# IBM/VillanDiffusion

Measured on AMD Instinct MI355X. Metric: train imgs/sec + 1000-step DDPM sample imgs/sec, CIFAR10 bs128, higher is better.
Workload: dtype bf16x3/f32; 1 GPU; DDPM-CIFAR10-32 poisoned fine-tune B=128 (BOX_14->HAT pr0.1 SDE-VP) + DDPM-1000 sampling 1024 img/GPU (8x128, 4 streams); global_batch=128, image=3x32x32, parallelism=dp1, mode=all, full=False

## Files before the change

include/villan_hip.h:

```cpp
#ifndef VILLAN_HIP_H
#define VILLAN_HIP_H

#include <stdint.h>

#ifdef __cplusplus
extern "C" {
#endif

#define VD_ABI_VERSION 11
#define VD_EINVAL (-22)
#define VD_ETIMEDOUT (-110)

int vd_abi_version(void);
const char* vd_last_error(void);
int vd_device_ok(void);
int vd_async_errors(int clear);

enum vd_a_mode { VD_A_ROW = 0,
                 VD_A_COL = 1 };
enum vd_b_mode { VD_B_PLAIN = 0,
                 VD_B_KCONTIG = 1,
                 VD_B_CONV3 = 2,
                 VD_B_CONV3_T = 3,
                 VD_B_CONV3_S2 = 4,
// ... 64 lines not shown
} vd_wgrad_desc;

int vd_conv_wgrad(const vd_wgrad_desc* desc, void* stream);
int64_t vd_conv_wgrad_ws_floats(const vd_wgrad_desc* desc);
int vd_conv_wgrad_plan(const vd_wgrad_desc* desc, int* tile, int* splits);

int vd_presplit_pack(const float* x, void* y, int B, int C, int HW, int64_t x_bstride, int64_t y_bstride, void* stream);
int vd_presplit_unpack(const void* y, float* x, int B, int C, int HW, int64_t y_bstride, int64_t x_bstride, void* stream);
int vd_groupnorm_fwd_presplit_ok(int C, int HW, int G);
int vd_groupnorm_fwd_presplit(const float* x, const float* gamma, const float* beta, void* y, float* mean, float* rstd, int B, int C, int HW, int G,
                              float eps, int apply_silu, int64_t x_bstride, int64_t y_bstride, void* stream);
int vd_groupnorm_bwd_presplit(const float* dy, const float* x, const float* mean, const float* rstd, const float* gamma, const float* beta,
                              const float* extra, const float* extra2, float* dx, void* dx_ps, float* dgamma_ws, float* dbeta_ws, float* rowsum,
                              int B, int C, int HW, int G, int apply_silu, int64_t dy_bstride, int64_t x_bstride, int64_t extra_bstride,
                              int64_t extra2_bstride, int64_t dx_bstride, int64_t ps_bstride, int64_t rowsum_ld, void* stream);

int vd_conv_wgrad_group_class(const vd_wgrad_desc* desc);
int64_t vd_conv_wgrad_group_job_bytes(void);
int vd_conv_wgrad_group_variant(int cls);
int vd_conv_wgrad_group_plan(const vd_wgrad_desc* descs, int n, void* table_out, int64_t* ws_floats, int* blocks, int* rblocks);
int vd_conv_wgrad_group_rebase(void* dev_table, int n, float* ws, void* stream);
int vd_conv_wgrad_group_launch(const void* dev_table, int n, int cls, int blocks, int rblocks, void* stream);

int64_t vd_conv3_packed_bytes(int M, int C, int taps);
int vd_conv3_pack_weights(const float* W, void* packed, int M, int C, int taps, int64_t row_stride, int64_t chan_stride, void* stream);
int vd_conv3_pack_weights_multi(const int64_t* table, int n_jobs, int64_t total_blocks, void* stream);
int vd_conv3_pack_weights_f16_multi(const int64_t* table, int n_jobs, int64_t total_blocks, void* stream);

int vd_weight_transpose(const float* W, float* Wt, int M, int C, int T, void* stream);
int vd_sumpool2x2(const float* dU, float* dX, int B, int C, int H, int W, int64_t du_bstride, int64_t dx_bstride,
                  int accumulate, void* stream);
int vd_col2im_s2(const float* G, float* dX, int B, int C, int H, int W, int OH, int OW, int pad, int64_t g_bstride,
                 int64_t dx_bstride, void* stream);
int vd_rowsum(const float* X, float* ws, int B, int M, int P, int64_t x_bstride, int64_t ws_ld, void* stream);
int vd_colsum(const float* ws, float* out, int B, int C, int64_t ld, int accumulate, void* stream);
int vd_colsum_segmented(const int64_t* table, int n_jobs, int B, void* stream);

int64_t vd_groupnorm_ws_floats(int B, int C, int HW, int G);
int vd_groupnorm_fwd(const float* x, const float* gamma, const float* beta, float* y, float* mean, float* rstd,
                     int B, int C, int HW, int G, float eps, int apply_silu, int64_t x_bstride, int64_t y_bstride,
                     float* ws, void* stream);
int vd_groupnorm_stats(const float* x, const float* gamma, const float* beta, float* ss, float* mean, float* rstd,
                       int B, int C, int HW, int G, float eps, int64_t x_bstride, void* stream);
int vd_groupnorm_stats_from_partials(const float* part, int tiles, const float* gamma, const float* beta, float* ss, float* mean,
                                     float* rstd, int B, int C, int HW, int G, float eps, void* stream);
int vd_groupnorm_bwd(const float* dy, const float* x, const float* mean, const float* rstd, const float* gamma,
                     const float* beta, const float* extra, float* dx, float* dgamma_ws, float* dbeta_ws,
                     int B, int C, int HW, int G, int apply_silu, int64_t dy_bstride, int64_t x_bstride,
                     int64_t extra_bstride, int64_t dx_bstride, float* ws, void* stream);
int vd_groupnorm_bwd_fused(const float* dy, const float* x, const float* mean, const float* rstd, const float* gamma,
                           const float* beta, const float* extra, const float* extra2, float* dx, float* dgamma_ws,
                           float* dbeta_ws, float* rowsum, int B, int C, int HW, int G, int apply_silu,
                           int64_t dy_bstride, int64_t x_bstride, int64_t extra_bstride, int64_t extra2_bstride,
                           int64_t dx_bstride, int64_t rowsum_ld, float* ws, void* stream);

int vd_softmax_col_fwd(float* S, int nb, int N, void* stream);
int vd_softmax_col_bwd(const float* P, float* dP, int nb, int N, float scale, void* stream);
int vd_attn_small_fwd(const float* qkv, float* out, float* P, int B, int C, int N, float scale,
                      int64_t qkv_bstride, int64_t out_bstride, void* stream);
int vd_attn_small_bwd(const float* qkv, const float* P, const float* dout, float* dqkv, int B, int C, int N,
                      float scale, int64_t qkv_bstride, int64_t dout_bstride, int64_t dqkv_bstride, void* stream);

int vd_attn_core_fwd(const float* qkv, float* out, float* P, int B, int heads, int head_dim, int N, float scale, void* stream);
int vd_attn_core_bwd(const float* qkv, const float* P, const float* out, const float* dout, float* dS, float* dqkv, int B, int heads,
                     int head_dim, int N, float scale, void* stream);

// ... 73 lines not shown
```

villandiffusion_amd/lib.py:

```python
from __future__ import annotations

import ctypes as C
import os
import subprocess
from typing import Optional

_HERE = os.path.dirname(os.path.abspath(__file__))
LIB_PATH = os.path.join(_HERE, "libvillan_hip.so")
CSRC = os.path.join(_HERE, "csrc")

A_ROW, A_COL = 0, 1
B_PLAIN, B_KCONTIG, B_CONV3, B_CONV3_T, B_CONV3_S2, B_CONV3_UP, B_CONV3_DIL, B_CONVG = range(8)

_i32, _i64, _f32, _vp = C.c_int32, C.c_int64, C.c_float, C.c_void_p


class GemmDesc(C.Structure):
    _fields_ = [("A", _vp), ("B", _vp), ("D", _vp), ("bias", _vp), ("rowadd", _vp), ("residual", _vp),
                ("M", _i32), ("N", _i32), ("K", _i32), ("a_mode", _i32), ("b_mode", _i32), ("NP", _i32),
                ("C", _i32), ("H", _i32), ("W", _i32), ("OH", _i32), ("OW", _i32),
                ("bias_on_n", _i32), ("d_trans", _i32), ("accumulate", _i32), ("tile", _i32), ("debug", _i32), ("alpha", _f32),
                ("lda", _i64), ("a_bstride", _i64), ("ldb", _i64), ("b_bstride", _i64),
                ("ldd", _i64), ("d_bstride", _i64), ("res_bstride", _i64), ("rowadd_bstride", _i64), ("ws", _vp), ("pad", _i32), ("nb2", _i32),
                ("a_b2stride", _i64), ("b_b2stride", _i64), ("d_b2stride", _i64), ("gn_ss", _vp), ("a_packed", _vp), ("a_packed_mpad", _i32), ("math", _i32), ("pool2", _i32),
# ... 8 lines not shown
                ("mode", _i32), ("splits", _i32), ("accumulate", _i32), ("tile", _i32),
                ("dy_bstride", _i64), ("x_bstride", _i64), ("pad", _i32), ("math", _i32), ("presplit", _i32), ("reserved_", _i32)]


PROTOTYPES = {
    "vd_abi_version": (_i32, []),
    "vd_last_error": (C.c_char_p, []),
    "vd_async_errors": (_i32, [_i32]),
    "vd_device_ok": (_i32, []),
    "vd_gemm": (_i32, [C.POINTER(GemmDesc), _vp]),
    "vd_gemm_tile": (_i32, [C.POINTER(GemmDesc)]),
    "vd_gemm_ws_floats": (_i64, [C.POINTER(GemmDesc)]),
    "vd_conv_wgrad": (_i32, [C.POINTER(WgradDesc), _vp]),
    "vd_conv_wgrad_plan": (_i32, [C.POINTER(WgradDesc), C.POINTER(_i32), C.POINTER(_i32)]),
    "vd_conv_wgrad_ws_floats": (_i64, [C.POINTER(WgradDesc)]),
    "vd_presplit_pack": (_i32, [_vp, _vp, _i32, _i32, _i32, _i64, _i64, _vp]),
    "vd_presplit_unpack": (_i32, [_vp, _vp, _i32, _i32, _i32, _i64, _i64, _vp]),
    "vd_groupnorm_fwd_presplit_ok": (_i32, [_i32, _i32, _i32]),
    "vd_groupnorm_fwd_presplit": (_i32, [_vp, _vp, _vp, _vp, _vp, _vp, _i32, _i32, _i32, _i32, _f32, _i32, _i64, _i64, _vp]),
    "vd_groupnorm_bwd_presplit": (_i32, [_vp] * 12 + [_vp, _i32, _i32, _i32, _i32, _i32] + [_i64] * 7 + [_vp]),
    "vd_conv_wgrad_group_class": (_i32, [C.POINTER(WgradDesc)]),
    "vd_conv_wgrad_group_job_bytes": (_i64, []),
    "vd_conv_wgrad_group_variant": (_i32, [_i32]),
    "vd_conv_wgrad_group_plan": (_i32, [C.POINTER(WgradDesc), _i32, _vp, C.POINTER(_i64), C.POINTER(_i32), C.POINTER(_i32)]),
    "vd_conv_wgrad_group_rebase": (_i32, [_vp, _i32, _vp, _vp]),
    "vd_conv_wgrad_group_launch": (_i32, [_vp, _i32, _i32, _i32, _i32, _vp]),
    "vd_conv3_packed_bytes": (_i64, [_i32, _i32, _i32]),
    "vd_conv3_pack_weights": (_i32, [_vp, _vp, _i32, _i32, _i32, _i64, _i64, _vp]),
    "vd_conv3_pack_weights_multi": (_i32, [_vp, _i32, _i64, _vp]),
    "vd_conv3_pack_weights_f16_multi": (_i32, [_vp, _i32, _i64, _vp]),
    "vd_weight_transpose": (_i32, [_vp, _vp, _i32, _i32, _i32, _vp]),
    "vd_sumpool2x2": (_i32, [_vp, _vp, _i32, _i32, _i32, _i32, _i64, _i64, _i32, _vp]),
    "vd_col2im_s2": (_i32, [_vp, _vp, _i32, _i32, _i32, _i32, _i32, _i32, _i32, _i64, _i64, _vp]),
    "vd_rowsum": (_i32, [_vp, _vp, _i32, _i32, _i32, _i64, _i64, _vp]),
    "vd_colsum": (_i32, [_vp, _vp, _i32, _i32, _i64, _i32, _vp]),
    "vd_colsum_segmented": (_i32, [_vp, _i32, _i32, _vp]),
    "vd_groupnorm_ws_floats": (_i64, [_i32, _i32, _i32, _i32]),
    "vd_groupnorm_stats": (_i32, [_vp, _vp, _vp, _vp, _vp, _vp, _i32, _i32, _i32, _i32, _f32, _i64, _vp]),
    "vd_groupnorm_fwd": (_i32, [_vp, _vp, _vp, _vp, _vp, _vp, _i32, _i32, _i32, _i32, _f32, _i32, _i64, _i64, _vp, _vp]),
    "vd_groupnorm_bwd": (_i32, [_vp] * 10 + [_i32] * 5 + [_i64] * 4 + [_vp, _vp]),
    "vd_groupnorm_stats_from_partials": (_i32, [_vp, _i32, _vp, _vp, _vp, _vp, _vp, _i32, _i32, _i32, _i32, _f32, _vp]),
    "vd_groupnorm_bwd_fused": (_i32, [_vp] * 12 + [_i32] * 5 + [_i64] * 6 + [_vp, _vp]),
    "vd_softmax_col_fwd": (_i32, [_vp, _i32, _i32, _vp]),
    "vd_softmax_col_bwd": (_i32, [_vp, _vp, _i32, _i32, _f32, _vp]),
    "vd_attn_small_fwd": (_i32, [_vp, _vp, _vp, _i32, _i32, _i32, _f32, _i64, _i64, _vp]),
    "vd_attn_small_bwd": (_i32, [_vp, _vp, _vp, _vp, _i32, _i32, _i32, _f32, _i64, _i64, _i64, _vp]),
    "vd_attn_core_fwd": (_i32, [_vp, _vp, _vp, _i32, _i32, _i32, _i32, _f32, _vp]),
    "vd_attn_core_bwd": (_i32, [_vp, _vp, _vp, _vp, _vp, _vp, _i32, _i32, _i32, _i32, _f32, _vp]),
    "vd_attn_flash_fwd": (_i32, [_vp, _vp, _vp, _i32, _i32, _i32, _i32, _f32, _i64, _i64, _vp]),
    "vd_attn_flash_bwd": (_i32, [_vp, _vp, _vp, _vp, _vp, _vp, _i32, _i32, _i32, _i32, _f32, _i64, _i64, _i64, _i64, _vp]),
    "vd_timestep_embedding": (_i32, [_vp, _vp, _vp, _i32, _i32, _i32, _vp]),
    "vd_silu_fwd": (_i32, [_vp, _vp, _i64, _vp]),
    "vd_silu_bwd": (_i32, [_vp, _vp, _vp, _i64, _i32, _vp]),
    "vd_add_strided": (_i32, [_vp, _vp, _i32, _i64, _i64, _i64, _i32, _vp]),
    "vd_scale": (_i32, [_vp, _i64, _f32, _vp]),
    "vd_lincomb": (_i32, [_vp, C.POINTER(_vp), C.POINTER(_f32), _i32, _i64, _vp]),
    "vd_qsample_backdoor": (_i32, [_vp] * 10 + [_i32, _i64, _vp]),
    "vd_mse_fwd_bwd": (_i32, [_vp] * 6 + [_i32, _i64, _f32, _vp]),
    "vd_loss_fwd_bwd": (_i32, [_vp] * 6 + [_i32, _i64, _f32, _i32, _vp]),
    "vd_trigger_inv_objective": (_i32, [_vp, _vp, _f32, _vp, _vp, _vp, _vp, _i32, _i64, _i64, _vp]),
    "vd_removal_loss": (_i32, [_vp, _vp, _f32, _f32, _f32, _vp, _vp, _vp, _i32, _i64, _i64, _vp]),
    "vd_score_inv_objective": (_i32, [_vp, _vp, _f32, _f32, _vp, _vp, _vp, _vp, _i32, _i64, _i64, _vp]),
    "vd_image_set_stats": (_i32, [_vp, _i32, _i32, _i32, _i32, _i64, _f32, _f32, _f32, _f32, _vp, _vp, _vp, _vp]),
    "vd_image_set_merge": (_i32, [_vp, _vp, _i64, _vp, _vp, _i64, _i64, _vp, _vp]),
    "vd_l2norm_sq": (_i32, [_vp, _i64, _vp, _vp, _vp]),
    "vd_adam_step": (_i32, [_vp, _vp, _vp, _vp, _i64, _vp, _f32, _f32, _f32, _f32, _f32, _f32, _i32, _vp, _vp]),
# ... 82 lines not shown
```

villandiffusion_amd/ops.py:

```python
from __future__ import annotations

import ctypes as C
import math
import os
from typing import Optional, Sequence

import torch

from . import lib as L
from .lib import (A_COL, A_ROW, B_CONV3, B_CONV3_DIL, B_CONVG, B_CONV3_S2, B_CONV3_T, B_CONV3_UP, B_KCONTIG, B_PLAIN,
                  GemmDesc, WgradDesc)


def _lib():
    L.require_device()
    return L.load()


_PROF = None

_B_NAMES = {0: "PLAIN", 1: "KCONTIG", 2: "CONV3", 3: "CONV3_T", 4: "CONV3_S2", 5: "CONV3_UP", 6: "CONV3_DIL", 7: "CONVG"}
_TILE_NAMES = {1: "128x128", 2: "64x128", 3: "64x64", 4: "patch128x128"}


# ... 651 lines not shown
        return (OH * OW) % 8 == 0 and M >= 64 and Cc >= 64
    if (mode == B_CONV3 and OW == 4 and OH == 4) or (mode in (B_CONV3, B_CONV3_UP) and OW >= 64 and OW % 32 == 0):
        return M >= 64 and Cc >= 64
    if mode == B_CONV3_S2:
        return OH == OW and (OW in (8, 16, 32) or (OW >= 64 and OW % 32 == 0)) and M >= 64 and Cc >= 64 and _wgrad_s2_split(OW)
    return mode in (B_CONV3, B_CONV3_UP) and OH == OW and OW in (8, 16, 32) and M >= 64 and Cc >= 64


def wgrad_ws_floats(M, Cc, T, nb, NP, OH=None, OW=None, mode=None, math_mode=0) -> int:
    d = WgradDesc()
    if OH is None:
        OH = OW = int(round(math.sqrt(NP)))
    d.M, d.C, d.T, d.nb, d.NP, d.OH, d.OW = M, Cc, T, nb, NP, OH, OW
    d.mode = (B_PLAIN if T == 1 else B_CONV3) if mode is None else mode
    d.math = math_mode
    scale = {B_CONV3_UP: (1, 2), B_CONV3_S2: (2, 1)}.get(d.mode, (1, 1))
    d.H, d.W = OH * scale[0] // scale[1], OW * scale[0] // scale[1]
    return int(L.load().vd_conv_wgrad_ws_floats(C.byref(d)))


def weight_transpose(w2d, wt, M, Cc, T):
    L.check(_lib().vd_weight_transpose(_p(w2d), _p(wt), M, Cc, T, _s()), "vd_weight_transpose")
    return wt


def sumpool2x2(dU, dX, accumulate=False):
    Bn, Cc, H, W, xbs = _img(dX)
    ubs = _img(dU)[4]
    assert dU.shape == (Bn, Cc, 2 * H, 2 * W)
    L.check(_lib().vd_sumpool2x2(_p(dU), _p(dX), Bn, Cc, H, W, ubs, xbs, int(accumulate), _s()), "vd_sumpool2x2")
    return dX


def conv3x3_s2_dgrad(dy, w2d, dx, pad=0, a_packed=None):
    Bn, M, OH, OW, dbs = _img(dy)
    Bx, Cc, H, W, xbs = _img(dx)
    assert Bx == Bn and w2d.shape == (M, Cc * 9) and w2d.is_contiguous()
    OHW = OH * OW
    G = torch.empty((Bn, Cc * 9, OHW), device=dy.device, dtype=torch.float32)
    gemm(w2d, dy, G, M=Cc * 9, N=Bn * OHW, K=M, a_mode=A_COL, b_mode=B_PLAIN, NP=OHW, lda=Cc * 9, ldb=OHW, b_bstride=dbs,
         ldd=OHW, d_bstride=Cc * 9 * OHW, a_packed=a_packed)
    L.check(_lib().vd_col2im_s2(_p(G), _p(dx), Bn, Cc, H, W, OH, OW, pad, Cc * 9 * OHW, xbs, _s()), "vd_col2im_s2")
    return dx


def rowsum(x, ws, ws_ld=None):
    Bn, M, H, W, xbs = _img(x)
    ld = M if ws_ld is None else ws_ld
    L.check(_lib().vd_rowsum(_p(x), _p(ws), Bn, M, H * W, xbs, ld, _s()), "vd_rowsum")
    return ws


def colsum(ws, out, Bn, Cc, ld=None, accumulate=False):
    L.check(_lib().vd_colsum(_p(ws), _p(out), Bn, Cc, Cc if ld is None else ld, int(accumulate), _s()), "vd_colsum")
    return out


def colsum_segmented(table, n_jobs, Bn):
    assert table.dtype == torch.int64 and table.is_contiguous() and table.numel() >= 4 * n_jobs
    L.check(_lib().vd_colsum_segmented(_p(table), n_jobs, Bn, _s()), "vd_colsum_segmented")


def _gn_ws(Bn, Cc, HW, G, device):
    need = _lib().vd_groupnorm_ws_floats(Bn, Cc, HW, G)
    return _gemm_ws(need, device) if need > 0 else None


def groupnorm_fwd(x, gamma, beta, y, mean, rstd, G, eps, silu):
    Bn, Cc, H, W, xbs = _img(x)
    ybs = _img(y)[4]
    assert y.shape == x.shape and mean.numel() >= Bn * G and rstd.numel() >= Bn * G
    _timed("groupnorm_fwd (gn_fwd_reg_kernel<*> / gn_chunk_*)", 8.0 * x.numel(), "hbm", lambda: L.check(
        _lib().vd_groupnorm_fwd(_p(x), _p(gamma), _p(beta), _p(y), _p(mean), _p(rstd), Bn, Cc, H * W, G, eps,
                                int(silu), xbs, ybs, _p(_gn_ws(Bn, Cc, H * W, G, x.device)), _s()), "vd_groupnorm_fwd"))
    return y
# ... 340 lines not shown
```

villandiffusion_amd/unet.py:

```python
from __future__ import annotations

import math
import os
from types import SimpleNamespace
from typing import Dict, List, Optional, Sequence, Tuple

import torch
import torch.nn as nn

from . import ops
from .lib import B_CONV3, B_CONV3_DIL, B_CONV3_S2, B_CONV3_T, B_CONV3_UP, B_PLAIN, A_COL, A_ROW, B_KCONTIG

LEGACY_ATTN = {"query": "to_q", "key": "to_k", "value": "to_v", "proj_attn": "to_out.0"}


class _Node(nn.Module):
    """Anonymous container used to reproduce diffusers' dotted state-dict names."""


def _ensure_path(root: nn.Module, parts: Sequence[str]) -> nn.Module:
    m = root
    for p in parts:
        if p not in m._modules:
            m.add_module(p, _Node())
# ... 111 lines not shown

def _wgrad1x1_math(net, dy, x) -> int:
    ok = _split(net) and ops.wgrad_bx3_eligible(dy.shape[1], x.shape[1], dy.shape[2], dy.shape[3], B_PLAIN) \
        and x.stride(0) % 4 == 0 and dy.stride(0) % 4 == 0
    return int(ok)


class _Conv:

    def __init__(self, net, prefix, cin, cout, mode=B_CONV3, pad=0):
        self.net, self.prefix, self.cin, self.cout, self.mode, self.pad = net, prefix, cin, cout, mode, pad
        net._decl(prefix + ".weight", (cout, cin, 3, 3), fan_in=cin * 9)
        net._decl(prefix + ".bias", (cout,), fan_in=cin * 9, is_bias=True)

    def w2d(self):
        return self.net.P[self.prefix + ".weight"].view(self.cout, self.cin * 9)

    def fwd(self, x, out, rowadd=None, rowadd_bstride=0, residual=None, gn_ss=None, gn_part=None):
        pk = _bx3_packed(self.net, self.prefix, False, self.cout, self.cin, out.shape[2], out.shape[3], self.mode)
        if gn_ss is not None and (out.shape[3] not in (16, 32) or self.mode != B_CONV3):
            pk = None
        return ops.conv3x3(x, self.w2d(), self.net.P[self.prefix + ".bias"], out, mode=self.mode, rowadd=rowadd,
                           rowadd_bstride=rowadd_bstride, residual=residual, pad=self.pad, gn_ss=gn_ss, a_packed=pk, gn_part=gn_part)

    def us_input(self, h, save):
        net = self.net
        B, _, H, W = h.shape
        if (self.mode != B_CONV3_UP or not net.us_fwd_presplit or not getattr(net, "presplit", False) or not _pairs(net) or H != W
                or not ops.conv_presplit_ok(B, self.cin, self.cout, 2 * H, 2 * W, B_CONV3_UP)
                or (save and not (net.group_wgrad and ops.wgrad_presplit_ok(B, self.cin, self.cout, 2 * H, B_CONV3_UP)))):
            return h
        return ops.presplit_pack(h)

    def bwd(self, dout, x, dx, bias_ws=None, skip_bias=False, dout_ps=None):
        net = self.net
        dout_f32 = dout
        if isinstance(x, ops.PreSplit):
            dy_ps = dout_ps if dout_ps is not None else net.pack_later(dout)
            net.wgrad(dy_ps, x, net.G[self.prefix + ".weight"].view(self.cout, self.cin * 9), self.mode, pad=self.pad, math_mode=1)
            if dout_ps is not None:
                dout = dout_ps
        elif (self.mode == B_CONV3_UP and getattr(net, "presplit", False) and _pairs(net) and net.group_wgrad
              and dout.shape[2] == dout.shape[3] and ops.wgrad_presplit_ok(dout.shape[0], self.cin, self.cout, dout.shape[3], B_CONV3_UP)):
            dy_ps = dout_ps if dout_ps is not None else net.pack_later(dout)
            net.wgrad(dy_ps, net.pack_later(x), net.G[self.prefix + ".weight"].view(self.cout, self.cin * 9), self.mode, pad=self.pad, math_mode=1)
        else:
            assert dout is not None
            bx3 = _split(net) and ops.wgrad_bx3_eligible(self.cout, self.cin, dout.shape[2], dout.shape[3],
                                                                                           self.mode) and x.stride(0) % 4 == 0
            net.wgrad(dout, x, net.G[self.prefix + ".weight"].view(self.cout, self.cin * 9), self.mode, pad=self.pad, math_mode=int(bx3))
        if not skip_bias:
            B = dout.shape[0]
            ws = bias_ws if bias_ws is not None else net.scratch_bc(B, self.cout)
            if bias_ws is None:
                assert dout_f32 is not None
                net.rowsum(dout_f32, ws)
            net.colsum_later(ws, net.G[self.prefix + ".bias"], B, self.cout, ld=(ws.stride(0) if ws.dim() == 2 else self.cout))
        if dx is None:
            return None
        if self.mode == B_CONV3_S2:
            pk = _bx3_packed_1x1(net, self.prefix + "::s2g", True, self.cin * 9, self.cout, dout.shape[2] * dout.shape[3], dout.shape[0])
            return ops.conv3x3_s2_dgrad(dout, self.w2d(), dx, pad=self.pad, a_packed=pk)
        pk = _bx3_packed(net, self.prefix, True, self.cin, self.cout, dout.shape[2], dout.shape[3], B_CONV3_T) \
            if self.mode in (B_CONV3, B_CONV3_UP) else None
        wt = net.wt_view(self.prefix, self.cout, self.cin, 9, fresh=pk is None)
        if self.mode == B_CONV3:
            ops.conv3x3(dout, wt, None, dx, mode=B_CONV3_T, a_packed=pk)
        elif self.mode == B_CONV3_UP:
            B, _, OH, OW = dout.shape
            if pk is not None and ops.bx3_pool2_eligible(self.cin, self.cout, OH, OW, B):
                src = dout_ps if (dout_ps is not None and net.us_dgrad_presplit and ops.conv_presplit_ok(B, self.cout, self.cin, OH, OW, B_CONV3_T)) else dout
                ops.conv3x3(src, wt, None, dx, mode=B_CONV3_T, a_packed=pk, pool2=True)
            else:
                dU = torch.empty((B, self.cin, OH, OW), device=dout.device, dtype=torch.float32)
                ops.conv3x3(dout, wt, None, dU, mode=B_CONV3_T, a_packed=pk)
                ops.sumpool2x2(dU, dx)
        else:
            raise NotImplementedError(self.mode)
        return dx


class _Norm:
    def __init__(self, net, prefix, ch, silu, groups=None):
        self.net, self.prefix, self.ch, self.silu = net, prefix, ch, silu
        self.groups = net.groups if groups is None else groups
        net._decl(prefix + ".weight", (ch,), ones=True)
        net._decl(prefix + ".bias", (ch,), zeros=True)

    def fwd(self, x, y):
        net = self.net
        B = x.shape[0]
        mean = torch.empty(B * self.groups, device=x.device, dtype=torch.float32)
        rstd = torch.empty_like(mean)
        ops.groupnorm_fwd(x, net.P[self.prefix + ".weight"], net.P[self.prefix + ".bias"], y, mean, rstd, self.groups,
                          net.eps, self.silu)
# ... 529 lines not shown
                self._wt_offs[name[:-7]] = wt_total
                wt_total += int(math.prod(shape))
        self._wt_offs["conv_in"] = wt_total
        wt_total += int(math.prod(offs["conv_in.weight"][2]))
        self._wt_total = wt_total
        self._wt_buf: Optional[torch.Tensor] = None
        self.wgrad_ws: Optional[torch.Tensor] = None
        self._cs_pool: Optional[torch.Tensor] = None
        self._cs_tables: Dict[tuple, torch.Tensor] = {}
        self._cs_cols_hint = 4 * sum(int(math.prod(sh)) for _, sh, _ in layout if len(sh) == 1) + 4096
        self._cs_off, self._cs_jobs, self._cs_B, self._cs_retired = 0, [], 0, []
        self._d_temb: Dict[int, torch.Tensor] = {}
        half = self.time_dim0 // 2
        exponent = -math.log(10000) * torch.arange(0, half, dtype=torch.float32)
        exponent = exponent / (half - self.config.freq_shift)
        self.freqs = torch.exp(exponent).to(dev)
        self._anchor = torch.zeros(1, device=dev, requires_grad=True)
        def _late(k):
            return ".time_emb_proj." in k or ".to_q." in k or ".to_k." in k or ".to_v." in k
        o_in = offs["conv_in.weight"][0]
        o_mid = min(v[0] for k, v in offs.items() if k.startswith("mid_block.") and not _late(k))
        o_up = min(v[0] for k, v in offs.items() if k.startswith("up_blocks.") and not _late(k))
        self.grad_buckets = [(o_up, total), (o_mid, o_up), (o_in, o_mid), (0, o_in)]
        self.bucket_ready_hook = None
        self.fuse_gn_inference = None
        self.fused_attention = os.environ.get("VILLAN_FUSED_ATTENTION", "1") != "0"
        self.sampler_graph = os.environ.get("VILLAN_SAMPLER_GRAPH", "1") != "0"
        self.group_wgrad = os.environ.get("VILLAN_GROUP_WGRAD", "1") != "0"
        self._wg_jobs: Dict[int, list] = {}
        self.wgrad_stream = os.environ.get("VILLAN_WGRAD_STREAM", "1") != "0"
        self.wgrad_flush_jobs = int(os.environ.get("VILLAN_WGRAD_FLUSH_JOBS", "24"))
        self._wg_side, self._wg_keep, self._rs_jobs = None, [], []
        self.fuse_gn_bwd = os.environ.get("VILLAN_FUSE_GN_BWD", "1") != "0"
        self.presplit = os.environ.get("VILLAN_PRESPLIT", "1") != "0"
        self.nograd_presplit = os.environ.get("VILLAN_NOGRAD_PRESPLIT", "1") != "0"
        self.us_dgrad_presplit = os.environ.get("VILLAN_US_DGRAD_PRESPLIT", "1") != "0"
        self.us_fwd_presplit = os.environ.get("VILLAN_US_FWD_PRESPLIT", "1") != "0"
        self.sc_stream = os.environ.get("VILLAN_SC_STREAM", "1") != "0"
        self._aux_stream = None
        self.gn_stats_in_epilogue = os.environ.get("VILLAN_GN_STATS_IN_EPILOGUE", "1") != "0"
        self._pk_jobs = []
        self.conv_math = CONV_MATH_DEFAULT
        self._packed: Optional[_PackedConvWeights] = None
        self._packed16: Optional[_PackedConvWeights] = None
        self._wt_fresh = set()
        self.reset_parameters()

    @torch.no_grad()
    def reset_parameters(self, seed: Optional[int] = None):
        gen = torch.Generator().manual_seed(seed) if seed is not None else None
        host = torch.zeros(self.flat_numel, dtype=torch.float32)
        for name, shape, meta in self._layout:
            off, n, _ = self._offs[name]
            if meta.get("ones"):
                host[off:off + n] = 1.0
            elif meta.get("zeros"):
                host[off:off + n] = 0.0
            else:
                bound = 1.0 / math.sqrt(meta["fan_in"])
                host[off:off + n] = (torch.rand(n, generator=gen) * 2 - 1) * bound
        self.flat_param.copy_(host)

    def zero_grad(self, set_to_none: bool = False):
        ops.scale_(self.flat_grad, 0.0)

    def load_state_dict(self, state_dict, strict: bool = True):
# ... 441 lines not shown
                elif len(sv) == st.marks["down_end"]:
                    self._bucket_boundary(1, hook)
            rec = sv.pop()
            kind = rec[0]
            if kind in ("res", "attn"):
                layer, saved = rec[1], rec[2]
                x = saved[0]
                is_cat_input = kind == "res" and any(x.data_ptr() == c.data_ptr() and x.shape == c.shape for c in st.cats)
                dx = torch.empty(x.shape, device=dev, dtype=torch.float32)
                rs = self.scratch_bc(B, x.shape[1]).view(B, x.shape[1]) if fuse else None
                dxp = wants_ps(layer.norm1 if kind == "res" else layer.norm, x.shape) if fuse else None
                if is_cat_input:
                    slot -= 1
                    dcats[slot] = dx
                    layer.bwd(saved, g, dx, st, dout_rs=g_rs, dx_rs=rs, dout_ps=g_ps, dx_ps=dxp)
                    g = dx[:, :up_slots[slot][0]]
                    g_rs = rs[:, :up_slots[slot][0]] if fuse else None
                    g_ps = dxp.channels(0, up_slots[slot][0]) if dxp is not None and up_slots[slot][0] % 8 == 0 else None
                elif fuse:
                    layer.bwd(saved, g, dx, st, dout_rs=g_rs, extra2=self._skip_grad(x, st, dcats), dx_rs=rs, dout_ps=g_ps, dx_ps=dxp)
                    g, g_rs, g_ps = dx, rs, dxp
                else:
                    layer.bwd(saved, g, dx, st, dout_ps=g_ps)
                    g, g_ps = dx, None
                    g = self._add_skip_grad(g, x, st, dcats)
            elif kind == "us":
                layer, x = rec[1], rec[2]
                dx = torch.empty(x.shape, device=dev, dtype=torch.float32)
                layer.bwd(g, x, dx, bias_ws=g_rs, dout_ps=g_ps)
                g, g_rs, g_ps = dx, None, None
            elif kind == "ds":
                layer, x = rec[1], rec[2]
                dx = torch.empty(x.shape, device=dev, dtype=torch.float32)
                layer.bwd(g, x, dx, bias_ws=g_rs)
                g, g_rs, g_ps = self._add_skip_grad(dx, x, st, dcats), None, None
            elif kind == "conv_in":
                if want_dx:
                    dx_in = torch.empty(rec[1].shape, device=dev, dtype=torch.float32)
                self._conv_in.bwd(g, rec[1], dx_in, bias_ws=g_rs)
            else:
                raise RuntimeError(kind)
        if not weights:
            return dx_in
        self._cs_flush()
        if hook is not None:
            hook(2)
        emb_sin, e1, e1a, emb, emb_act = st.temb_saved
        d = st.d_temb_all
        ops.linear_wgrad(d, emb_act, self.gWt_all, accumulate=True)
        self.colsum_later(d, self.gbt_all, B, self.temb_total)
        d_act = torch.empty_like(emb_act)
        ops.linear_dgrad(d, self.Wt_all, d_act)
        d_emb = ops.silu_bwd(d_act, emb, torch.empty_like(emb))
        ops.linear_wgrad(d_emb, e1a, self.G["time_embedding.linear_2.weight"], accumulate=True)
        ops.colsum(d_emb, self.G["time_embedding.linear_2.bias"], B, self.temb_dim, accumulate=True)
        d_e1a = torch.empty_like(e1a)
        ops.linear_dgrad(d_emb, self.P["time_embedding.linear_2.weight"], d_e1a)
        d_e1 = ops.silu_bwd(d_e1a, e1, torch.empty_like(e1))
        ops.linear_wgrad(d_e1, emb_sin, self.G["time_embedding.linear_1.weight"], accumulate=True)
        ops.colsum(d_e1, self.G["time_embedding.linear_1.bias"], B, self.temb_dim, accumulate=True)
        self._cs_flush()
        if hook is not None:
            hook(3)
        return dx_in

    def _skip_grad(self, x, st, dcats):
        for k, c in enumerate(st.cats):
            h_ch = st.up_slots[k][0]
# ... 10 lines not shown
```

Baseline: 7598 train images/s.

## Fuse stride-2 conv dgrad GEMM, col2im, skip-grad add and rowsum into one kernel

Adds a HIP kernel for the backward data gradient of stride-2 3x3 downsample convolutions. It computes the bf16x3 MFMA GEMM, folds the col2im scatter in shared memory, adds the skip-connection gradient, and emits per-channel rowsums for the next bias gradient in one pass. This replaces a GEMM that wrote a 9x-expanded intermediate G, plus separate col2im, skip-add and rowsum launches. The cost is a complex tiling (14 channels per tile, 256 pixels) restricted to square 4/8/16 outputs, with extra shared-memory epilogue work and possible tile underutilisation.

```diff
diff --git a/include/villan_hip.h b/include/villan_hip.h
--- a/include/villan_hip.h
+++ b/include/villan_hip.h
@@ -120,6 +120,9 @@
                   int accumulate, void* stream);
 int vd_col2im_s2(const float* G, float* dX, int B, int C, int H, int W, int OH, int OW, int pad, int64_t g_bstride,
                  int64_t dx_bstride, void* stream);
+int vd_conv3x3_s2_dgrad_fused(const float* dY, const void* a_packed, float* dX, const float* skip, float* rowsum, int B, int cin, int cout,
+                              int OH, int OW, int pad, int64_t dy_bstride, int64_t dx_bstride, int64_t skip_bstride, int64_t rowsum_ld,
+                              void* stream);
 int vd_rowsum(const float* X, float* ws, int B, int M, int P, int64_t x_bstride, int64_t ws_ld, void* stream);
 int vd_colsum(const float* ws, float* out, int B, int C, int64_t ld, int accumulate, void* stream);
 int vd_colsum_segmented(const int64_t* table, int n_jobs, int B, void* stream);
diff --git a/villandiffusion_amd/csrc/vd_s2_dgrad.hip b/villandiffusion_amd/csrc/vd_s2_dgrad.hip
--- /dev/null
+++ b/villandiffusion_amd/csrc/vd_s2_dgrad.hip
@@ -0,0 +1,263 @@
+#include "vd_common.h"
+
+namespace {
+
+typedef __bf16 bf16x8 __attribute__((ext_vector_type(8)));
+typedef unsigned int u32x4 __attribute__((ext_vector_type(4)));
+
+constexpr int XC = 16;
+constexpr int GS = 4;
+constexpr int S2F_CH = 7;
+constexpr int S2F_TILE_CH = 2 * S2F_CH;
+
+__device__ __forceinline__ void split_bf16x8(const float (&v)[8], u32x4& hi, u32x4& lo) {
+    bf16x8 h, l;
+#pragma unroll
+    for (int j = 0; j < 8; ++j) {
+        const __bf16 t = (__bf16)v[j];
+        h[j] = t;
+        l[j] = (__bf16)(v[j] - (float)t);
+    }
+    hi = __builtin_bit_cast(u32x4, h);
+    lo = __builtin_bit_cast(u32x4, l);
+}
+
+__device__ __forceinline__ int bswz(int n) {
+    const int a = (n >> 2) & 7, b = n & 3;
+    return (n & ~31) | (((a + 2 * b) & 7) + 8 * (a >> 2) + 16 * ((a >> 1) & 1));
+}
+
+struct s2f_args {
+    const float* dY;
+    const u32x4* Apk;
+    float* dX;
+    const float* sg;
+    float* rs;
+    int B, cin, cout, pad, M, Mpad;
+    int64_t dy_bs, dx_bs, sg_bs, rs_ld;
+};
+
+template <int OW>
+__global__ __launch_bounds__(512, 2) void s2_dgrad_bx3_kernel(const s2f_args a) {
+    constexpr int NTH = 512, WM = 2, WN = 2, BM = 128, BN = 256, WAVES_N = 4;
+    constexpr int A_IT = GS * 4 * BM / NTH;
+    constexpr int NP = OW * OW, W = 2 * OW, HW = 4 * NP, IMGS = BN / NP;
+    constexpr int GLD = BN + 4;
+    constexpr int HALF = S2F_CH * BN * 4;
+    __shared__ u32x4 smem[GS * 4 * BM + GS * 4 * BN];
+    u32x4* __restrict__ As = smem;
+    u32x4* __restrict__ Bs = smem + GS * 4 * BM;
+    float* __restrict__ Gs = reinterpret_cast<float*>(smem);
+    float* __restrict__ Ds = Gs + 64 * GLD;
+    static_assert((64 * GLD + HALF) * 4 <= (int)sizeof(smem), "epilogue buffers exceed the stage buffers");
+
+    const int tid = threadIdx.x, lane = tid & 63, wave = tid >> 6, h = lane >> 5, l31 = lane & 31;
+    const int tiles_m = (a.cin + S2F_TILE_CH - 1) / S2F_TILE_CH;
+    int bid = blockIdx.x;
+    {
+        const int nwg = gridDim.x;
+        if ((nwg & 7) == 0) bid = (bid & 7) * (nwg >> 3) + (bid >> 3);
+    }
+    const int tm = bid % tiles_m, tn = bid / tiles_m;
+    const int n0 = tn * BN, N = a.B * NP;
+    const int Mpad = a.Mpad;
+    const int nchunks = a.cout / XC;
+    const int nst = (nchunks + GS - 1) / GS;
+    const int pg = tid & (BN / 4 - 1), pq = (tid / (BN / 4)) & 1, psub = tid / (BN / 2);
+    const int b_first = tn * IMGS;
+    const __amdgpu_buffer_rsrc_t brs = __builtin_amdgcn_make_buffer_rsrc(const_cast<float*>(a.dY + (int64_t)b_first * a.dy_bs), 0, 0xFFFFFFF0, 0x00020000);
+    const __amdgpu_buffer_rsrc_t ars = __builtin_amdgcn_make_buffer_rsrc(const_cast<u32x4*>(a.Apk), 0, 0xFFFFFFF0, 0x00020000);
+    unsigned bpix;
+    {
+        const int n = min(n0 + 4 * pg, N - 4);
+        const int b = n / NP;
+        bpix = 4u * (unsigned)((b - b_first) * a.dy_bs + (n - b * NP) + (int64_t)pq * 8 * NP);
+    }
+    const unsigned ldb4 = 4u * (unsigned)NP;
+    const int r_lds = tid & 127;
+    const int a_row = min(tm * (2 * S2F_CH * 9) + r_lds - (r_lds >= 64 ? 1 : 0), a.M - 1);
+    const unsigned a_lane = 16u * (unsigned)((tid >> 7) * Mpad + a_row);
+
+    u32x4 ra0[A_IT], ra1[A_IT];
+    f32x4 rp0[8], rp1[8];
+    auto load_stage = [&](int st, u32x4 (&ra)[A_IT], f32x4 (&rp)[8]) {
+        const int cc0 = min(st, nst - 1) * GS;
+#pragma unroll
+        for (int i = 0; i < A_IT; ++i) {
+            const int cc = min(cc0 + i, nchunks - 1);
+            ra[i] = __builtin_bit_cast(u32x4, __builtin_amdgcn_raw_buffer_load_b128(ars, a_lane, 16u * (unsigned)(cc * 4 * Mpad), 0));
+        }
+        {
+            const int cc = min(cc0 + psub, nchunks - 1);
+            const unsigned vo = bpix + (unsigned)(cc * XC) * ldb4;
+#pragma unroll
+            for (int j = 0; j < 8; ++j) rp[j] = __builtin_bit_cast(f32x4, __builtin_amdgcn_raw_buffer_load_b128(brs, vo, j * ldb4, 0));
+        }
+    };
+    auto store_stage = [&](const u32x4 (&ra)[A_IT], const f32x4 (&rp)[8]) {
+#pragma unroll
+        for (int i = 0; i < A_IT; ++i) As[tid + i * NTH] = ra[i];
+#pragma unroll
+        for (int px = 0; px < 4; ++px) {
+            float w[8];
+#pragma unroll
+            for (int j = 0; j < 8; ++j) w[j] = rp[j][px];
+            u32x4 hi, lo;
+            split_bf16x8(w, hi, lo);
+            Bs[((psub * 2 + 0) * 2 + pq) * BN + bswz(4 * pg + px)] = hi;
+            Bs[((psub * 2 + 1) * 2 + pq) * BN + bswz(4 * pg + px)] = lo;
+        }
+    };
+
+    f32x16 acc[WM][WN];
+#pragma unroll
+    for (int mi = 0; mi < WM; ++mi)
+#pragma unroll
+        for (int ni = 0; ni < WN; ++ni)
+#pragma unroll
+            for (int v = 0; v < 16; ++v) acc[mi][ni][v] = 0.f;
+
+    const int wm = wave / WAVES_N, wn = wave % WAVES_N;
+    const u32x4* __restrict__ a_base = As + h * BM + wm * 64 + l31;
+    const u32x4* __restrict__ b_base = Bs + h * BN + wn * 64 + bswz(l31);
+    auto mfma_stage = [&](int st) {
+#pragma unroll
+        for (int sub = 0; sub < GS; ++sub) {
+            if (st * GS + sub < nchunks) {
+                bf16x8 ah[WM], al[WM];
+#pragma unroll
+                for (int mi = 0; mi < WM; ++mi) {
+                    ah[mi] = __builtin_bit_cast(bf16x8, a_base[(sub * 4 + 0) * BM + mi * 32]);
+                    al[mi] = __builtin_bit_cast(bf16x8, a_base[(sub * 4 + 2) * BM + mi * 32]);
+                }
+#pragma unroll
+                for (int ni = 0; ni < WN; ++ni) {
+                    const bf16x8 bh = __builtin_bit_cast(bf16x8, b_base[(sub * 4 + 0) * BN + ni * 32]);
+                    const bf16x8 bl = __builtin_bit_cast(bf16x8, b_base[(sub * 4 + 2) * BN + ni * 32]);
+#pragma unroll
+                    for (int mi = 0; mi < WM; ++mi) {
+                        acc[mi][ni] = __builtin_amdgcn_mfma_f32_32x32x16_bf16(al[mi], bh, acc[mi][ni], 0, 0, 0);
+                        acc[mi][ni] = __builtin_amdgcn_mfma_f32_32x32x16_bf16(ah[mi], bl, acc[mi][ni], 0, 0, 0);
+                        acc[mi][ni] = __builtin_amdgcn_mfma_f32_32x32x16_bf16(ah[mi], bh, acc[mi][ni], 0, 0, 0);
+                    }
+                }
+            }
+        }
+    };
+
+    load_stage(0, ra0, rp0);
+    load_stage(1, ra1, rp1);
+    store_stage(ra0, rp0);
+    __syncthreads();
+    for (int st = 0; st < nst; st += 2) {
+        load_stage(st + 2, ra0, rp0);
+        mfma_stage(st);
+        __syncthreads();
+        store_stage(ra1, rp1);
+        __syncthreads();
+        if (st + 1 >= nst) break;
+        load_stage(st + 3, ra1, rp1);
+        mfma_stage(st + 1);
+        __syncthreads();
+        store_stage(ra0, rp0);
+        __syncthreads();
+    }
+
+    constexpr int EPT = HALF / NTH;
+    float sgv[2][EPT];
+#pragma unroll
+    for (int hm = 0; hm < 2; ++hm)
+#pragma unroll
+        for (int i = 0; i < EPT; ++i) {
+            const int e = tid + i * NTH;
+            const int k = e / (IMGS * HW), rem = e - k * (IMGS * HW);
+            const int img = rem / HW, pix = rem - img * HW;
+            const int c = tm * S2F_TILE_CH + hm * S2F_CH + k, b = b_first + img;
+            sgv[hm][i] = (a.sg != nullptr && c < a.cin && b < a.B) ? a.sg[(int64_t)b * a.sg_bs + (int64_t)c * HW + pix] : 0.f;
+        }
+
+#pragma unroll
+    for (int hm = 0; hm < 2; ++hm) {
+        if (hm == 1) __syncthreads();
+        if (wm == hm) {
+#pragma unroll
+            for (int mi = 0; mi < WM; ++mi)
+#pragma unroll
+                for (int ni = 0; ni < WN; ++ni)
+#pragma unroll
+                    for (int v = 0; v < 16; ++v)
+                        Gs[(mi * 32 + (v & 3) + 8 * (v >> 2) + 4 * h) * GLD + wn * 64 + ni * 32 + l31] = acc[mi][ni][v];
+        }
+        __syncthreads();
+        const int c0 = tm * S2F_TILE_CH + hm * S2F_CH;
+#pragma unroll
+        for (int i = 0; i < EPT; ++i) {
+            const int e = tid + i * NTH;
+            const int k = e / (IMGS * HW), rem = e - k * (IMGS * HW);
+            const int img = rem / HW, pix = rem - img * HW;
+            const int y = pix / W, x = pix - y * W;
+            const float* __restrict__ g = Gs + (k * 9) * GLD + img * NP;
+            const int yp = y + a.pad, xp = x + a.pad;
+            const int r0 = yp & 1, s0 = xp & 1;
+            float v = 0.f;
+#pragma unroll
+            for (int jr = 0; jr < 2; ++jr) {
+                const int r = r0 + 2 * jr, iy = (yp - r) >> 1;
+                const bool rok = r < 3 && yp >= r && iy < OW;
+#pragma unroll
+                for (int js = 0; js < 2; ++js) {
+                    const int sx = s0 + 2 * js, ix = (xp - sx) >> 1;
+                    const bool ok = rok && sx < 3 && xp >= sx && ix < OW;
+                    const float t = g[ok ? (r * 3 + sx) * GLD + iy * OW + ix : 0];
+                    v += ok ? t : 0.f;
+                }
+            }
+            const int c = c0 + k, b = b_first + img;
+            if (a.sg != nullptr) v = v + sgv[hm][i];
+            if (c < a.cin && b < a.B) a.dX[(int64_t)b * a.dx_bs + (int64_t)c * HW + pix] = v;
+            if (a.rs != nullptr) Ds[e] = v;
+        }
+        if (a.rs != nullptr) {
+            __syncthreads();
+            for (int p = wave; p < S2F_CH * IMGS; p += NTH / 64) {
+                const float* __restrict__ dp = Ds + p * HW;
+                float s = 0.f;
+                for (int j = lane; j < HW; j += 64) s += dp[j];
+                s = wave_sum(s);
+                const int k = p / IMGS, img = p - k * IMGS;
+                const int c = c0 + k, b = b_first + img;
+                if (lane == 0 && c < a.cin && b < a.B) a.rs[(int64_t)b * a.rs_ld + c] = s;
+            }
+        }
+    }
+}
+
+}
+
+extern "C" int vd_conv3x3_s2_dgrad_fused(const float* dY, const void* a_packed, float* dX, const float* skip, float* rowsum, int B, int cin, int cout,
+                                         int OH, int OW, int pad, int64_t dy_bstride, int64_t dx_bstride, int64_t skip_bstride, int64_t rowsum_ld,
+                                         void* stream) {
+    VD_REQUIRE(dY && a_packed && dX && B > 0 && cin > 0 && cout > 0, "vd_conv3x3_s2_dgrad_fused: bad args");
+    VD_REQUIRE(OH == OW && (OW == 4 || OW == 8 || OW == 16), "vd_conv3x3_s2_dgrad_fused: square 4x4 / 8x8 / 16x16 outputs only (OH=%d OW=%d)", OH, OW);
+    VD_REQUIRE(pad == 0 || pad == 1, "vd_conv3x3_s2_dgrad_fused: pad must be 0 or 1");
+    VD_REQUIRE(cout % XC == 0, "vd_conv3x3_s2_dgrad_fused: cout %% 16 != 0 (cout=%d)", cout);
+    const int NP = OH * OW, imgs = 256 / NP;
+    const int64_t chw_out = (int64_t)cout * NP, chw_in = (int64_t)cin * 4 * NP;
+    VD_REQUIRE(dy_bstride >= chw_out && (dy_bstride & 3) == 0 && ((((uintptr_t)dY) | ((uintptr_t)a_packed)) & 15) == 0,
+               "vd_conv3x3_s2_dgrad_fused: dY needs 16-byte alignment and a batch stride that is a multiple of 4 floats");
+    VD_REQUIRE(dx_bstride >= chw_in && (!skip || skip_bstride >= chw_in) && (!rowsum || rowsum_ld >= cin), "vd_conv3x3_s2_dgrad_fused: bad strides");
+    const int M = cin * 9, Mpad = (M + 127) / 128 * 128;
+    VD_REQUIRE(((int64_t)(imgs - 1) * dy_bstride + chw_out) * 4 < (1ll << 31) && (int64_t)Mpad * cout * 4 < (1ll << 31) && (int64_t)B * NP < (1ll << 30),
+               "vd_conv3x3_s2_dgrad_fused: operand too large for 32-bit offsets");
+    s2f_args a;
+    a.dY = dY, a.Apk = reinterpret_cast<const u32x4*>(a_packed), a.dX = dX, a.sg = skip, a.rs = rowsum;
+    a.B = B, a.cin = cin, a.cout = cout, a.pad = pad, a.M = M, a.Mpad = Mpad;
+    a.dy_bs = dy_bstride, a.dx_bs = dx_bstride, a.sg_bs = skip_bstride, a.rs_ld = rowsum_ld;
+    const int grid = vd_cdiv(cin, S2F_TILE_CH) * vd_cdiv((int64_t)B * NP, 256);
+    hipStream_t st = (hipStream_t)stream;
+    if (OW == 16) hipLaunchKernelGGL(s2_dgrad_bx3_kernel<16>, dim3(grid), dim3(512), 0, st, a);
+    else if (OW == 8) hipLaunchKernelGGL(s2_dgrad_bx3_kernel<8>, dim3(grid), dim3(512), 0, st, a);
+    else hipLaunchKernelGGL(s2_dgrad_bx3_kernel<4>, dim3(grid), dim3(512), 0, st, a);
+    VD_LAUNCH_CHECK("vd_conv3x3_s2_dgrad_fused");
+    return 0;
+}
diff --git a/villandiffusion_amd/lib.py b/villandiffusion_amd/lib.py
--- a/villandiffusion_amd/lib.py
+++ b/villandiffusion_amd/lib.py
@@ -64,6 +64,7 @@
     "vd_weight_transpose": (_i32, [_vp, _vp, _i32, _i32, _i32, _vp]),
     "vd_sumpool2x2": (_i32, [_vp, _vp, _i32, _i32, _i32, _i32, _i64, _i64, _i32, _vp]),
     "vd_col2im_s2": (_i32, [_vp, _vp, _i32, _i32, _i32, _i32, _i32, _i32, _i32, _i64, _i64, _vp]),
+    "vd_conv3x3_s2_dgrad_fused": (_i32, [_vp] * 5 + [_i32] * 6 + [_i64] * 4 + [_vp]),
     "vd_rowsum": (_i32, [_vp, _vp, _i32, _i32, _i32, _i64, _i64, _vp]),
     "vd_colsum": (_i32, [_vp, _vp, _i32, _i32, _i64, _i32, _vp]),
     "vd_colsum_segmented": (_i32, [_vp, _i32, _i32, _vp]),
diff --git a/villandiffusion_amd/ops.py b/villandiffusion_amd/ops.py
--- a/villandiffusion_amd/ops.py
+++ b/villandiffusion_amd/ops.py
@@ -707,15 +707,56 @@
     return dX
 
 
-def conv3x3_s2_dgrad(dy, w2d, dx, pad=0, a_packed=None):
+S2F_TILE_CH = 14
+
+
+def s2_dgrad_tile_rows(cin: int):
+    M = cin * 9
+    tiles = []
+    for tm in range((cin + S2F_TILE_CH - 1) // S2F_TILE_CH):
+        rows = []
+        for r in range(128):
+            half, k = r // 64, (r % 64) // 9
+            gathered = (r % 64) < 63 and tm * S2F_TILE_CH + half * 7 + k < cin
+            rows.append((min(tm * 126 + r - (1 if r >= 64 else 0), M - 1), gathered))
+        tiles.append(rows)
+    return tiles
+
+
+def s2_dgrad_fused_ok(a_packed, cout, OH, OW, H, W, dy_bstride, dy_addr=0, packed_addr=0) -> bool:
+    if a_packed is None or a_packed is False or isinstance(a_packed, tuple):
+        return False
+    if cout <= 0 or cout % 16 != 0 or OH != OW or OW not in (4, 8, 16) or H != 2 * OH or W != 2 * OW:
+        return False
+    if dy_bstride % 4 != 0 or dy_addr % 16 != 0 or packed_addr % 16 != 0:
+        return False
+    return (((256 // (OH * OW)) - 1) * dy_bstride + cout * OH * OW) * 4 < 2 ** 31
+
+
+def conv3x3_s2_dgrad(dy, w2d, dx, pad=0, a_packed=None, skip=None, rowsum=None, fused=True):
     Bn, M, OH, OW, dbs = _img(dy)
     Bx, Cc, H, W, xbs = _img(dx)
     assert Bx == Bn and w2d.shape == (M, Cc * 9) and w2d.is_contiguous()
     OHW = OH * OW
+    if skip is not None:
+        assert tuple(skip.shape) == tuple(dx.shape)
+    if rowsum is not None:
+        assert tuple(rowsum.shape) == (Bn, Cc) and (Cc == 1 or rowsum.stride(1) == 1)
+    rs_ld = 0 if rowsum is None else (rowsum.stride(0) if Bn > 1 else Cc)
+    if fused and s2_dgrad_fused_ok(a_packed, M, OH, OW, H, W, dbs, dy.data_ptr(), 0 if a_packed is None or isinstance(a_packed, tuple) else a_packed.data_ptr()):
+        sbs = _img(skip)[4] if skip is not None else 0
+        _timed(f"s2_dgrad_bx3_kernel<{OW}>", 2.0 * Cc * 9 * M * Bn * OHW, "mfma", lambda: L.check(
+            _lib().vd_conv3x3_s2_dgrad_fused(_p(dy), _p(a_packed), _p(dx), _p(skip), _p(rowsum), Bn, Cc, M, OH, OW, pad, dbs, xbs, sbs, rs_ld, _s()),
+            "vd_conv3x3_s2_dgrad_fused"), nbytes=4.0 * (dy.numel() + dx.numel() * (2 if skip is not None else 1)))
+        return dx
     G = torch.empty((Bn, Cc * 9, OHW), device=dy.device, dtype=torch.float32)
     gemm(w2d, dy, G, M=Cc * 9, N=Bn * OHW, K=M, a_mode=A_COL, b_mode=B_PLAIN, NP=OHW, lda=Cc * 9, ldb=OHW, b_bstride=dbs,
          ldd=OHW, d_bstride=Cc * 9 * OHW, a_packed=a_packed)
     L.check(_lib().vd_col2im_s2(_p(G), _p(dx), Bn, Cc, H, W, OH, OW, pad, Cc * 9 * OHW, xbs, _s()), "vd_col2im_s2")
+    if skip is not None:
+        add_strided(dx, skip, accumulate=True)
+    if rowsum is not None:
+        L.check(_lib().vd_rowsum(_p(dx), _p(rowsum), Bn, Cc, H * W, xbs, rs_ld, _s()), "vd_rowsum")
     return dx
 
 
diff --git a/villandiffusion_amd/unet.py b/villandiffusion_amd/unet.py
--- a/villandiffusion_amd/unet.py
+++ b/villandiffusion_amd/unet.py
@@ -167,7 +167,16 @@
             return h
         return ops.presplit_pack(h)
 
-    def bwd(self, dout, x, dx, bias_ws=None, skip_bias=False, dout_ps=None):
+    def s2_fused_ok(self, dout, dx) -> bool:
+        net = self.net
+        if self.mode != B_CONV3_S2 or not getattr(net, "s2_dgrad_fused", False) or not isinstance(dout, torch.Tensor):
+            return False
+        pk = _bx3_packed_1x1(net, self.prefix + "::s2g", True, self.cin * 9, self.cout, dout.shape[2] * dout.shape[3], dout.shape[0])
+        if pk is None or isinstance(pk, tuple):
+            return False
+        return ops.s2_dgrad_fused_ok(pk, self.cout, dout.shape[2], dout.shape[3], dx.shape[2], dx.shape[3], ops._img(dout)[4], dout.data_ptr(), pk.data_ptr())
+
+    def bwd(self, dout, x, dx, bias_ws=None, skip_bias=False, dout_ps=None, s2_fused=False, skip=None, dx_rs=None):
         net = self.net
         dout_f32 = dout
         if isinstance(x, ops.PreSplit):
@@ -195,7 +204,8 @@
             return None
         if self.mode == B_CONV3_S2:
             pk = _bx3_packed_1x1(net, self.prefix + "::s2g", True, self.cin * 9, self.cout, dout.shape[2] * dout.shape[3], dout.shape[0])
-            return ops.conv3x3_s2_dgrad(dout, self.w2d(), dx, pad=self.pad, a_packed=pk)
+            assert s2_fused or (skip is None and dx_rs is None)
+            return ops.conv3x3_s2_dgrad(dout, self.w2d(), dx, pad=self.pad, a_packed=pk, skip=skip, rowsum=dx_rs, fused=s2_fused)
         pk = _bx3_packed(net, self.prefix, True, self.cin, self.cout, dout.shape[2], dout.shape[3], B_CONV3_T) \
             if self.mode in (B_CONV3, B_CONV3_UP) else None
         wt = net.wt_view(self.prefix, self.cout, self.cin, 9, fresh=pk is None)
@@ -791,6 +801,7 @@
         self.wgrad_flush_jobs = int(os.environ.get("VILLAN_WGRAD_FLUSH_JOBS", "24"))
         self._wg_side, self._wg_keep, self._rs_jobs = None, [], []
         self.fuse_gn_bwd = os.environ.get("VILLAN_FUSE_GN_BWD", "1") != "0"
+        self.s2_dgrad_fused = os.environ.get("VILLAN_S2_DGRAD_FUSED", "1") != "0"
         self.presplit = os.environ.get("VILLAN_PRESPLIT", "1") != "0"
         self.nograd_presplit = os.environ.get("VILLAN_NOGRAD_PRESPLIT", "1") != "0"
         self.us_dgrad_presplit = os.environ.get("VILLAN_US_DGRAD_PRESPLIT", "1") != "0"
@@ -1298,8 +1309,13 @@
             elif kind == "ds":
                 layer, x = rec[1], rec[2]
                 dx = torch.empty(x.shape, device=dev, dtype=torch.float32)
-                layer.bwd(g, x, dx, bias_ws=g_rs)
-                g, g_rs, g_ps = self._add_skip_grad(dx, x, st, dcats), None, None
+                if layer.s2_fused_ok(g, dx):
+                    rs = self.scratch_bc(B, x.shape[1]).view(B, x.shape[1]) if fuse and not self._dx_only else None
+                    layer.bwd(g, x, dx, bias_ws=g_rs, s2_fused=True, skip=self._skip_grad(x, st, dcats), dx_rs=rs)
+                    g, g_rs, g_ps = dx, rs, None
+                else:
+                    layer.bwd(g, x, dx, bias_ws=g_rs)
+                    g, g_rs, g_ps = self._add_skip_grad(dx, x, st, dcats), None, None
             elif kind == "conv_in":
                 if want_dx:
                     dx_in = torch.empty(rec[1].shape, device=dev, dtype=torch.float32)
```

After: 7664 train images/s (median of 6 runs). Within noise of the previous version (+0.9%).
